# CRIMAC-WP4-Machine-learning/CRIMAC-classifiers-unet

Measured on AMD Instinct MI355X. Metric: echogram patches/sec (4ch 256x256), training step (fwd+weighted CE+bwd+SGD), higher is better.
Workload: dtype bf16; 1 GPU; BASELINE configs[1]: U-Net (depth 5, 64 filters) train step, batch 32 x 4x256x256 per GPU; global_batch=32, precision=bf16, start_filts=64, parallelism=dp1, ranks=1, launcher=single process

## Files before the change

crimac_classifiers_unet_amd/csrc/common.h:

```cpp
#pragma once
#include <hip/hip_runtime.h>
#include <stdint.h>
#include <stdio.h>

#include "../../include/crimac_unet_hip.h"

typedef __bf16 bf16_t;
typedef _Float16 half_t;
typedef _Float16 half8 __attribute__((ext_vector_type(8)));
typedef __bf16 bf16x4 __attribute__((ext_vector_type(4)));
typedef __bf16 bf16x8 __attribute__((ext_vector_type(8)));
typedef unsigned short u16x4 __attribute__((ext_vector_type(4)));
typedef unsigned short u16x8 __attribute__((ext_vector_type(8)));
typedef float f32x4 __attribute__((ext_vector_type(4)));
typedef float f32x16 __attribute__((ext_vector_type(16)));
typedef unsigned int u32x4 __attribute__((ext_vector_type(4)));
typedef unsigned int u32x2 __attribute__((ext_vector_type(2)));

#define LDS_PTR(T) __attribute__((address_space(3))) T*

void crimac_set_error(const char* fmt, ...);
#define CRIMAC_REQUIRE(cond, ...)                 \
  do {                                            \
    if (!(cond)) {                                \
// ... 219 lines not shown
    for (int i = 0; i < 4; ++i) { v[i] = a[i]; v[4 + i] = b[i]; }
  }
#else
  load8(p, v);
#endif
}
__device__ __forceinline__ void store8(bf16_t* p, const float (&v)[8]) {
  u16x8 r;
#pragma unroll
  for (int i = 0; i < 8; ++i) r[i] = f2bfbits(v[i]);
  *reinterpret_cast<u16x8*>(p) = r;
}
__device__ __forceinline__ void store8(half_t* p, const float (&v)[8]) {
  half8 r;
#pragma unroll
  for (int i = 0; i < 8; ++i) r[i] = (half_t)v[i];
  *reinterpret_cast<half8*>(p) = r;
}
__device__ __forceinline__ void store8(float* p, const float (&v)[8]) {
  f32x4 a, b;
#pragma unroll
  for (int i = 0; i < 4; ++i) { a[i] = v[i]; b[i] = v[4 + i]; }
  *reinterpret_cast<f32x4*>(p) = a;
  *reinterpret_cast<f32x4*>(p + 4) = b;
}

__device__ __forceinline__ void store8(hp_t* p, const float (&v)[8]) {
  u32x4 h, l;
  hp_split(v, h, l);
  *reinterpret_cast<u32x4*>(p) = h;
  *(reinterpret_cast<u32x4*>(p) + 1) = l;
}

__device__ __forceinline__ float wave_sum(float v) {
#pragma unroll
  for (int o = 32; o > 0; o >>= 1) v += __shfl_xor(v, o, 64);
  return v;
}
__device__ __forceinline__ double wave_sum_d(double v) {
#pragma unroll
  for (int o = 32; o > 0; o >>= 1) v += __shfl_xor(v, o, 64);
  return v;
}

static inline bool crimac_first_use_on_device(unsigned long long* mask) {
  int dev = 0;
  if (hipGetDevice(&dev) != hipSuccess || dev < 0 || dev >= 64) return true;
  const unsigned long long bit = 1ull << dev;
  return (__atomic_fetch_or(mask, bit, __ATOMIC_ACQ_REL) & bit) == 0;
}
static inline int crimac_cu_count() {
  static int ncu[64] = {0};
  int dev = 0;
  if (hipGetDevice(&dev) != hipSuccess || dev < 0 || dev >= 64) return 256;
  int n = __atomic_load_n(&ncu[dev], __ATOMIC_RELAXED);
  if (n <= 0) {
    hipDeviceProp_t prop;
    n = (hipGetDeviceProperties(&prop, dev) == hipSuccess && prop.multiProcessorCount > 0) ? prop.multiProcessorCount : 256;
    __atomic_store_n(&ncu[dev], n, __ATOMIC_RELAXED);
  }
  return n;
}

#ifdef CRIMAC_DIAG_CLOCK
#define CRIMAC_DIAG_SLOTS 4096
#define CRIMAC_DIAG_DECLARE(name)                                                                   \
// ... 22 lines not shown
```

crimac_classifiers_unet_amd/csrc/elementwise.hip:

```cpp
#include <stdarg.h>
#include <stdlib.h>

#include <mutex>

#include "common.h"

static thread_local char g_err[512] = "";
void crimac_set_error(const char* fmt, ...) {
  va_list ap;
  va_start(ap, fmt);
  vsnprintf(g_err, sizeof(g_err), fmt, ap);
  va_end(ap);
}
extern "C" const char* crimac_last_error(void) { return g_err; }
extern "C" int crimac_version(void) { return CRIMAC_ABI_VERSION; }
extern "C" int crimac_layer_desc_size(void) { return (int)sizeof(crimac_layer_desc); }

namespace {

#ifdef CRIMAC_STREAM_FORWARD
#define CRIMAC_ROW(x, M) (x)
#else
#define CRIMAC_ROW(x, M) ((M) - 1 - (x))
#endif
// ... 813 lines not shown
    load8s(dp + r * dp_ld + c0, g);
    long pix[4];
#pragma unroll
    for (int d = 0; d < 4; ++d) {
      pix[d] = (b * H + 2 * yp + (d >> 1)) * (long)W + 2 * xp + (d & 1);
      load8s(y + pix[d] * y_ld + c0, yv[d]);
#pragma unroll
      for (int j = 0; j < 8; ++j) av[d][j] = storage_round<TA>(fmaxf(yv[d][j] * sc[j] + sh[j], 0.f));
    }
    int arg[8];
#pragma unroll
    for (int j = 0; j < 8; ++j) {
      int best = 0;
      float bv = av[0][j];
#pragma unroll
      for (int d = 1; d < 4; ++d)
        if (av[d][j] > bv) { bv = av[d][j]; best = d; }
      arg[j] = best;
    }
#pragma unroll
    for (int d = 0; d < 4; ++d) {
      float o[8];
      if (ds) load8s(ds + pix[d] * ds_ld + c0, o);
#pragma unroll
      for (int j = 0; j < 8; ++j) {
        const float dav = storage_round<T>((ds ? o[j] : 0.f) + (arg[j] == d ? g[j] : 0.f));
        o[j] = bn_bwd_dy(yv[d][j], dav, sc[j], sh[j], mu[j], is[j], k1[j], k2[j]);
      }
      store8(dy + pix[d] * dy_ld + c0, o);
    }
  }
}

template <typename T, int NC, typename TR = T>
__global__ __launch_bounds__(256) void head_fwd_kernel(const T* __restrict__ x, long x_ld, int Cin,
                                                       const float* __restrict__ w,
                                                       const float* __restrict__ bias,
                                                       float* __restrict__ logits, long npix, long HW,
                                                       int softmax, const float* __restrict__ bn_scale,
                                                       const float* __restrict__ bn_shift) {
  const int lp = Cin / 8;
  const int sub = threadIdx.x % lp;
  float bsc[8], bsh[8];
#pragma unroll
  for (int j = 0; j < 8; ++j) {
    bsc[j] = bn_scale ? bn_scale[sub * 8 + j] : 1.f;
    bsh[j] = bn_scale ? bn_shift[sub * 8 + j] : 0.f;
  }
  float wr[NC][8];
#pragma unroll
  for (int o = 0; o < NC; ++o)
#pragma unroll
    for (int j = 0; j < 8; ++j) wr[o][j] = w[o * Cin + sub * 8 + j];
  const long ppb = 256 / lp;
  for (long p0 = (long)blockIdx.x * ppb; p0 < npix; p0 += (long)gridDim.x * ppb) {
    const long p = p0 + threadIdx.x / lp;
    float acc[NC];
#pragma unroll
    for (int o = 0; o < NC; ++o) acc[o] = 0.f;
    if (p < npix) {
      float v[8];
      load8(x + p * x_ld + sub * 8, v);
      if (bn_scale) {
#pragma unroll
        for (int j = 0; j < 8; ++j) v[j] = storage_round<TR>(fmaxf(v[j] * bsc[j] + bsh[j], 0.f));
      }
// ... 685 lines not shown
  CRIMAC_LAUNCH_CHECK();
  return CRIMAC_OK;
}

extern "C" int crimac_unpool_bn_bwd_apply_replicas(int prec, const void* dp, long dp_ld, const void* ds, long ds_ld,
                                                   const void* y, long y_ld, const float* bn_vec, long bn_stride,
                                                   const double* sum_dz, const double* sum_dz_xhat, int replicas,
                                                   long count, void* dy, long dy_ld, int B, int H, int W, int C,
                                                   float* dgamma, float* dbeta, void* stream) {
  PREC_OK_BWD16("unpool_bn_bwd_apply_replicas");
  CRIMAC_REQUIRE(dp && y && bn_vec && bn_stride >= C && sum_dz && sum_dz_xhat && replicas >= 1 && dy && dgamma && dbeta &&
                     B > 0 && H > 0 && W > 0 && H % 2 == 0 && W % 2 == 0 && C > 0 && C % 8 == 0 && C <= 2048,
                 "unpool_bn_bwd_apply_replicas: bad arguments");
  const long M = (long)B * H * W;
  CRIMAC_REQUIRE(count == 0 || count >= M, "unpool_bn_bwd_apply_replicas: count smaller than the pixels of this call");
  if (count == 0) count = M;
  CRIMAC_REQUIRE(dp_ld >= C && y_ld >= C && dy_ld >= C && (!ds || ds_ld >= C) && dp_ld % 8 == 0 && y_ld % 8 == 0 &&
                     dy_ld % 8 == 0 && (!ds || ds_ld % 8 == 0),
                 "unpool_bn_bwd_apply_replicas: bad pixel strides");
  const long total = (long)B * (H / 2) * (W / 2) * (C / 8);
  const int grid = grid_for(total, 256 * 4);
  const size_t lds = 512 * sizeof(double) + 2 * (size_t)C * sizeof(float);
#define UBA(T, TD, TA)                                                                                                  \
  hipLaunchKernelGGL((unpool_bn_bwd_apply_kernel<T, TD, TA>), dim3(whole_rounds(unpool_bn_bwd_apply_kernel<T, TD, TA>, lds, grid)), dim3(256), lds, ST, (const T*)dp, dp_ld,      \
                     (const T*)ds, ds_ld, (const T*)y, y_ld, bn_vec + 2 * bn_stride, bn_vec + 3 * bn_stride, bn_vec,    \
                     bn_vec + bn_stride, sum_dz, sum_dz_xhat, replicas, count, (TD*)dy, dy_ld, B, H, W, C, dgamma, dbeta)
  if (prec == CRIMAC_PREC_H3F_BWD) UBA(float, half_t, hp_t);
  else CRIMAC_FOR_STORAGE2(prec, T, TP, UBA(T, TP, TP));
#undef UBA
  CRIMAC_LAUNCH_CHECK();
  return CRIMAC_OK;
}

template <typename T, typename TR = T>
static int head_fwd_launch(const void* x, long x_ld, int Cin, const float* w, const float* b,
                           float* logits, long npix, long HW, int ncls, int softmax, const float* bn_scale,
                           const float* bn_shift, hipStream_t st) {
  const int lp = Cin / 8;
  if (Cin == 64) {
    const int grid64 = grid_for(npix, 256 * 4);
#define HF64(NC)                                                                                              \
  hipLaunchKernelGGL((head_fwd64_kernel<T, NC, TR>), dim3(whole_rounds(head_fwd64_kernel<T, NC, TR>, 0, grid64)), dim3(256), 0, st, (const T*)x, x_ld, w, b, logits, \
                     npix, HW, softmax, bn_scale, bn_shift)
    if (ncls == 2) HF64(2); else if (ncls == 3) HF64(3); else HF64(4);
#undef HF64
    CRIMAC_LAUNCH_CHECK();
    return CRIMAC_OK;
  }
  const int grid = grid_for(npix, (256 / lp) * 8);
#define HF(NC)                                                                                      \
  hipLaunchKernelGGL((head_fwd_kernel<T, NC, TR>), dim3(whole_rounds(head_fwd_kernel<T, NC, TR>, 0, grid)), dim3(256), 0, st, (const T*)x, x_ld, Cin, \
                     w, b, logits, npix, HW, softmax, bn_scale, bn_shift)
  if (ncls == 2) HF(2); else if (ncls == 3) HF(3); else HF(4);
#undef HF
  CRIMAC_LAUNCH_CHECK();
  return CRIMAC_OK;
}

static bool head_cin_ok(int Cin) {
  const int lp = Cin / 8;
  return Cin > 0 && Cin % 8 == 0 && lp <= 64 && (lp & (lp - 1)) == 0;
}

extern "C" int crimac_head_fwd(int prec, const void* x, long x_ld, int Cin, const float* w,
                               const float* b, float* logits, int B, int H, int W, int ncls,
                               int softmax, const float* bn_scale, const float* bn_shift, void* stream) {
// ... 137 lines not shown
```

crimac_classifiers_unet_amd/csrc/wgrad.hip:

```cpp
#include "common.h"

CRIMAC_DIAG_DECLARE(crimac_diag_clock_wgrad)

namespace {

struct WgradParams {
  const void* f; long f_ld; int CF;
  const void* s; long s_ld; int CS;
  int B, Hf, Wf;
  float* dw;
  int tiles_y, tiles_x;
  long ntiles;
  int tiles_per_block;
  int nsplits;
  long partial_stride;
  int f_es = 2, s_es = 2;
};

__device__ __forceinline__ int swz_tr(int row) { return ((row >> 1) & 1) << 6; }

__device__ __forceinline__ bf16x4 lds_tr16(const unsigned char* p) {
  return __builtin_amdgcn_ds_read_tr16_b64_v4bf16((LDS_PTR(bf16x4))(p));
}


template <int OFF>
__device__ __forceinline__ bf16x4 lds_tr16_asm(unsigned addr) {
  bf16x4 v;
  asm volatile("ds_read_b64_tr_b16 %0, %1 offset:%2" : "=v"(v) : "v"(addr), "n"(OFF) : "memory");
  return v;
}
template <int N> __device__ __forceinline__ void wait_lgkm() {
  asm volatile("s_waitcnt lgkmcnt(%0)" :: "n"(N) : "memory");
}
__device__ __forceinline__ void tie(bf16x4& x) { asm volatile("" : "+v"(x)); }

__device__ __forceinline__ int swz16(int row) { return (((row >> 1) & 1) << 6) | (((row >> 2) & 1) << 5); }

template <int MODE, int TG>
struct WgTaps {
  static constexpr int TR = MODE == 0 ? 8 : 4;
  static constexpr int NRP = TR / 2;
  static constexpr int RS = MODE == 0 ? 18 : 64;
  static constexpr int T0 = MODE == 0 ? (TG == 0 ? 0 : 5) : (TG == 0 ? 0 : 2);
  static constexpr int N = MODE == 0 ? (TG == 0 ? 5 : 4) : 2;
  static constexpr int srow(int py, int t) {
    return MODE == 0 ? (py + t / 3) * 18 + t % 3 : (2 * py + (t >> 1)) * 32 + (t & 1) * 16;
  }
};
struct WgFrags {
  bf16x4 a[4][2];
  bf16x4 b[2][2][2];
};
template <int RP, int FH>
__device__ __forceinline__ void wg_rd_a(unsigned fv0, WgFrags& f) {
  f.a[FH][0] = lds_tr16_asm<(RP * 32) * 128>(fv0 ^ (FH << 5));
// ... 916 lines not shown
  if (col < 0) {
#else
  if (col < p.CS) {
#endif
    float* dwp = p.dw + (p.partial_stride > 0 ? (long)split * p.partial_stride : 0);
#pragma unroll
    for (int t = 0; t < NTAPS; ++t) {
#pragma unroll
      for (int r = 0; r < 16; ++r) {
        const int row = cf0 + wf * 32 + (r & 3) + 8 * (r >> 2) + 4 * (lane >> 5);
        if (row < p.CF) {
          float* dst = dwp + ((long)t * p.CF + row) * p.CS + col;
          if (p.partial_stride > 0) *dst = acc[t][r];
          else atomicAdd(dst, acc[t][r]);
        }
      }
    }
  }
}

constexpr int kGroupMaxLayers = CRIMAC_WGRAD_GROUP_MAX_LAYERS;
using GroupLayer = crimac_wgrad_group_layer;
struct GroupParams {
  GroupLayer layer[kGroupMaxLayers];
  int B;
  const int* items;
  int cap;
  int count[8];
  unsigned* counter;
  int f_es, s_es;
  int max_items;
};

__device__ __forceinline__ void group_barrier_lds() {
  asm volatile("s_waitcnt lgkmcnt(0)" ::: "memory");
  __builtin_amdgcn_s_barrier();
  asm volatile("" ::: "memory");
}

__device__ __forceinline__ unsigned lds_word(const unsigned* p) {
  return *(volatile LDS_PTR(unsigned))(LDS_PTR(unsigned))(p);
}

template <typename TA>
__global__ __launch_bounds__(512) __attribute__((amdgpu_waves_per_eu(2, 2)))
void wgrad_group_kernel(GroupParams gp) {
  constexpr int MODE = 0, TR = 8, NTAPS = 9;
  constexpr int F_ROWS = TR * 16;
  constexpr int S_ROWS = (TR + 2) * 18;
  constexpr int S_ROWS_PAD = (S_ROWS + 7) / 8 * 8;
  constexpr int F_BYTES = F_ROWS * 128;
  constexpr int S_BYTES = S_ROWS_PAD * 128;
  constexpr int BUF_BYTES = F_BYTES + S_BYTES;
  constexpr int NF = F_ROWS / 8 / 4;
  constexpr int NS = (S_ROWS_PAD / 8 + 3) / 4;
  constexpr unsigned OOB = 0x80000000u;
  extern __shared__ __attribute__((aligned(16))) unsigned char smem[];
  const int tid = threadIdx.x, lane = tid & 63;
  const int team = __builtin_amdgcn_readfirstlane(tid >> 8);
  const int wave = __builtin_amdgcn_readfirstlane((tid >> 6) & 3);
  const int ws = wave & 1, tg = wave >> 1;
  const int g = lane >> 4, li = lane & 15;
  const int q = li >> 2, pp = li & 3;
  const int sub = lane >> 3, c = lane & 7;
  const int xcd = blockIdx.x & 7;
  unsigned* tq = reinterpret_cast<unsigned*>(smem + 4 * BUF_BYTES);
  const int n_items = gp.count[xcd];
  auto fetch_item = [&](int par) {
    const unsigned k = __hip_atomic_fetch_add(gp.counter + xcd, 1u, __ATOMIC_RELAXED, __HIP_MEMORY_SCOPE_AGENT);
    unsigned a = 0, b = 0;
    if (k < (unsigned)n_items) {
// ... 649 lines not shown
```

crimac_classifiers_unet_amd/engine.py:

```python
from __future__ import annotations

import ctypes as C
import os

import torch

from . import hip
from .hip import Act, call, ptr


def _on_device(fn):
    import functools

    @functools.wraps(fn)
    def wrapped(self, *a, **kw):
        if getattr(self, "device", None) is None:
            self.bind()
        dev = self.device
        if dev is None or dev.type != "cuda":
            return fn(self, *a, **kw)
        with torch.cuda.device(dev):
            return fn(self, *a, **kw)
    return wrapped

# ... 409 lines not shown
            return
        arr, bounds = self._layer_table()
        done = getattr(self, "_packed_groups", set())
        if done:
            for gi in range(len(bounds)):
                if gi not in done:
                    self._pack_group(gi)
        elif len(arr):
            call("crimac_pack_layers", C.byref(arr), len(arr), self._fwd_planes_arg())
            if self.bwd16:
                call("crimac_pack_layers", C.byref(self._ltab16), len(arr), hip.PLANES_FP16)
        self._packed_groups = set()
        self._train_pack_dirty = False

    wgrad_side_streams = int(os.environ.get("CRIMAC_WGRAD_STREAM", "1"))
    early_sgd = True
    early_sgd_multi = os.environ.get("CRIMAC_EARLY_SGD_MULTI", "0") != "0"
    exchange_probe = None
    exchange_on_side = os.environ.get("CRIMAC_EXCHANGE_SIDE", "0") != "0"
    _side = None
    _side_events = None
    _eval_side = None

    @staticmethod
    def _gloo_ranks():
        import torch.distributed as dist
        return (dist.is_available() and dist.is_initialized() and dist.get_world_size() > 1
                and dist.get_backend() == "gloo")

    wgrad_group = True
    wgrad_group_h3p = False
    wgrad_group_layers = hip.WGRAD_GROUP_MAX_LAYERS
    _wg_pending = None

    def _groupable(self, prec, mode, cf, cs):
        if not (self.wgrad_group and mode == 0 and cs >= 64 and cf >= 64 and not self.use_wgrad_partials and self._wg_pending is not None):
            return False
        if prec == hip.PREC_H3P:
            return self.wgrad_group_h3p and cf % 64 == 0 and cs % 64 == 0
        return prec in hip.PREC_16BIT or prec == hip.PREC_H3F_BWD

    def _group_plan(self, B, shapes):
        key = (self.prec_bwd, B, shapes)
        plan = self._wg_plans.get(key)
        if plan is None:
            lib = hip.load_library()
            arr = (hip.WgradGroupLayer * len(shapes))()
            for d, (cf, cs, h, w, f_ld, s_ld) in zip(arr, shapes):
                d.CF, d.CS, d.Hf, d.Wf, d.f_ld, d.s_ld = cf, cs, h, w, f_ld, s_ld
            counts = (C.c_int * 8)()
            cap = lib.crimac_wgrad_group_plan(self.prec_bwd, arr, len(shapes), B, 0, None, 0, counts)
            if cap < 0:
                raise hip.HipLibraryError("crimac_wgrad_group_plan failed: " + lib.crimac_last_error().decode(errors="replace"))
            items = torch.zeros(8 * max(cap, 1) * 2, dtype=torch.int32)
            rc = lib.crimac_wgrad_group_plan(self.prec_bwd, arr, len(shapes), B, 0, C.c_void_p(items.data_ptr()), max(cap, 1),
                                             counts)
            if rc < 0:
                raise hip.HipLibraryError("crimac_wgrad_group_plan failed: " + lib.crimac_last_error().decode(errors="replace"))
            plan = (arr, items.to(self.device), counts, max(cap, 1))
            self._wg_plans[key] = plan
        return plan

    def _flush_wgrad_group(self):
        pend = self._wg_pending
        if not pend:
            return
# ... 130 lines not shown
        if t is None or tuple(t.shape) != tuple(shape) or t.dtype != dtype:
            t = torch.empty(shape, dtype=dtype, device=self.device)
            self._bufs[key] = t
        return t

    def _wfrag_geometry(self, B, H, W):
        es = 4 if self.is_hp else 2
        small = (B * H * W - 1) * (2 * self.sf) * es + 2 * self.sf * es < (1 << 31)
        if small == getattr(self, "_wfrag_on", True):
            return
        self._wfrag_on = small
        for pks in (self.pk_main, self.pk_eval, self.pk16):
            for key, pk in pks.items():
                ok = pk.get("frag_ok") or (self.pk_main.get(key, {}).get("frag_ok", (False, False)) if pks is self.pk_eval else None)
                if ok is None:
                    continue
                if "fwd_frag" in pk:
                    pk["fwd_frag"] = bool(small and ok[0])
                if "dg_frag" in pk:
                    pk["dg_frag"] = bool(small and ok[1])
        self._ltab = self._ltab16 = None
        self._packed_groups = set()
        self._train_pack_dirty = self._eval_pack_dirty = True

    def _geom(self, B, H, W):
        self._wfrag_geometry(B, H, W)
        D = self.depth
        if H % (2 ** (D - 1)) or W % (2 ** (D - 1)):
            raise ValueError(f"H, W must be divisible by {2 ** (D - 1)} (got {H}x{W})")
        return [(H >> i, W >> i, B * (H >> i) * (W >> i)) for i in range(D)]

    fuse_bn_bwd = True
    fuse_unpool_apply = None
    fuse_head_bn = True

    def _conv3x3(self, x: Act, pk, bias, out: Act, B, H, W, cin, cout, relu, dgrad=False, cin_real=None,
                 stats=None, bnb=None, cols=None, out_planes=False, stat_reps=None):
        flops = 2.0 * 9 * (cin_real or cin) * cout * B * H * W
        relu = (hip.EPI_RELU if relu else 0) | (hip.EPI_OUT_PLANES if (out_planes and self.is_hp) else 0)
        if pk.get("narrow"):
            return self._conv3x3_narrow(x, pk, bias, out, B, H, W, cin, cout, relu, dgrad, stats, cols, stat_reps, flops)
        if self.is_hp and cin_real is not None and cin_real <= 4 and cin == CIN_PAD and not dgrad:
            relu |= hip.EPI_CIN4
        w_hi, w_lo = ptr(pk["dg_hi" if dgrad else "fwd_hi"]), ptr(pk["dg_lo" if dgrad else "fwd_lo"])
        if pk.get("dg_frag" if dgrad else "fwd_frag"):
            relu |= hip.EPI_WFRAG
        prec = self.prec_bwd if dgrad else self.prec
        mode, s0, s1, by, by_ld, bvec = 0, None, None, None, 0, None
        reps = stat_reps or self._nrep(cout)
        if stats is not None:
            mode, s0, s1 = 1, ptr(stats[0]), ptr(stats[1])
        elif bnb is not None and self.fuse_bn_bwd:
            blk, y = bnb
            mode, s0, s1 = 2, ptr(self._stat(blk, 0)), ptr(self._stat(blk, 1))
            by, by_ld, bvec = y.p, y.ld, ptr(self._bnf(blk, 0))
        if cols is not None:
            call("crimac_conv3x3_cols", prec, x.p, x.ld, B, H, W, cin, cout, w_hi, w_lo, ptr(bias),
                 out.p, out.ld, relu, mode, s0, s1, reps, by, by_ld, bvec, self.cmax,
                 cols[0], cols[1], flops=flops * cols[1] / cout, mfmas=hip.MFMAS_PER_PRODUCT[prec])
            return mode != 0
        call("crimac_conv3x3", prec, x.p, x.ld, B, H, W, cin, cout, w_hi, w_lo, ptr(bias),
             out.p, out.ld, relu, mode, s0, s1, reps, by, by_ld, bvec, self.cmax,
             flops=flops, mfmas=hip.MFMAS_PER_PRODUCT[prec])
        return mode != 0

    def _conv3x3_narrow(self, x: Act, pk, bias, out: Act, B, H, W, cin, cout, flags, dgrad, stats, cols, stat_reps, flops):
# ... 329 lines not shown
            w64, wm = self._lmi_weights()
            call("crimac_head_fwd", self.prec, cur.p, cur.ld, self.sf, ptr(w64), ptr(self.P["conv_final.bias"]),
                 ptr(logits), B, H, W, self.n_classes, 0,
                 ptr(self._bnf(head_bn, 2)) if head_bn is not None else None,
                 ptr(self._bnf(head_bn, 3)) if head_bn is not None else None)
            m = self._buf("lmi.m", (B * H * W,), torch.float32)
            call("crimac_meta_mlp_fwd", ptr(meta), self.meta_channels, B, H, W, *self._mlp(), ptr(m))
            call("crimac_meta_inject_fwd", ptr(m), ptr(wm), ptr(logits), B, H, W, self.n_classes, 1 if softmax else 0)
            saved["meta"] = meta
        else:
            call("crimac_head_fwd", self.prec, cur.p, cur.ld, self.sf, ptr(self.P["conv_final.weight"]),
                 ptr(self.P["conv_final.bias"]), ptr(logits), B, H, W, self.n_classes, 1 if softmax else 0,
                 ptr(self._bnf(head_bn, 2)) if head_bn is not None else None,
                 ptr(self._bnf(head_bn, 3)) if head_bn is not None else None)
        saved["head_in"] = cur if head_bn is None else None
        self.saved = saved if training else None
        if training:
            self.forward_generation += 1
        return logits

    def _block_bwd(self, tag, b, da: Act, y: Act, x_in: Act, B, h, w, M, dx_out: Act, reduce_done=False,
                   next_bn=None, bias_from_stats=None, unpool_src=None):
        world = self._sync_world()
        folded = reduce_done and self.fold_bn_finalize and world == 1
        if folded:
            pass
        elif reduce_done:
            call("crimac_sum_replicas", ptr(self._stat(b, 0)), self._nrep(b.cout), b.cout, b.cout,
                 ptr(self._stat(b, 2)), None, ptr(self._stat(b, 1)), ptr(self._stat(b, 3)))
        else:
            call("crimac_bn_bwd_reduce", self.prec, da.p, da.ld, y.p, y.ld, ptr(self._bnf(b, 2)),
                 ptr(self._bnf(b, 3)), ptr(self._bnf(b, 0)), ptr(self._bnf(b, 1)), M, b.cout,
                 ptr(self._stat(b, 2)), ptr(self._stat(b, 3)))
        dy = Act(self._buf(f"{tag}.dy", (M, b.cout), torch.float16 if self.bwd16 else None), b.cout)
        prec_apply = self.prec_bwd if self.bwd16 else self.prec
        dgamma, dbeta = self.G[b.bn_key + ".weight"], self.G[b.bn_key + ".bias"]
        if world > 1:
            import torch.distributed as dist
            dgamma.copy_(self._stat(b, 3))
            dbeta.copy_(self._stat(b, 2))
            dist.all_reduce(self._stat_pair(b), group=UNetEngine._bn_group)
            scr = self._buf("g.syncbn.scratch", (2, self.cmax), torch.float32)
            dgamma, dbeta = scr[0], scr[1]
        if unpool_src is not None:
            if not folded:
                raise RuntimeError("unpool_src needs the folded BatchNorm-backward path")
            dp_, ds_ = unpool_src
            call("crimac_unpool_bn_bwd_apply_replicas", prec_apply, dp_.p, dp_.ld, ds_.p if ds_ is not None else None,
                 ds_.ld if ds_ is not None else 0, y.p, y.ld, ptr(self._bnf(b, 0)), self.cmax, ptr(self._stat(b, 0)),
                 ptr(self._stat(b, 1)), self._nrep(b.cout), M, dy.p, dy.ld, B, h, w, b.cout, ptr(dgamma), ptr(dbeta))
        elif folded:
            call("crimac_bn_bwd_apply_replicas", prec_apply, da.p, da.ld, y.p, y.ld, ptr(self._bnf(b, 0)), self.cmax,
                 ptr(self._stat(b, 0)), ptr(self._stat(b, 1)), self._nrep(b.cout), M, M, b.cout, dy.p, dy.ld,
                 ptr(dgamma), ptr(dbeta))
        else:
            call("crimac_bn_bwd_apply", prec_apply, da.p, da.ld, y.p, y.ld, ptr(self._bnf(b, 2)),
                 ptr(self._bnf(b, 3)), ptr(self._bnf(b, 0)), ptr(self._bnf(b, 1)), ptr(self._stat(b, 2)),
                 ptr(self._stat(b, 3)), M, M * world, b.cout, dy.p, dy.ld, ptr(dgamma), ptr(dbeta), None)
        self._wgrad(self.prec_bwd, 0, dy.p, dy.ld, b.cout, x_in.p, x_in.ld, b.cin_pad, B, h, w, b.conv_key,
                    flops=2.0 * 9 * b.cin * b.cout * B * h * w)
        fused = False
        if dx_out is not None:
            stats = None
            if bias_from_stats is not None:
                per = 2 * STAT_REPLICAS * 2 * self.cmax
                lvl = bias_from_stats[2]
# ... 81 lines not shown

    def _enc_group(self, i):
        return min(self.depth - i, self.n_enc_groups)

    def grad_ranges(self):
        if getattr(self, "_granges", None) is not None and self._granges[0] is self.layout:
            return self._granges[1]
        r = self._grad_ranges()
        self._granges = (self.layout, r)
        return r

    def _grad_ranges(self):
        dec = self.ups[0].key.split(".")[0] + "."
        lo_dec = min(o for k, (o, _, _) in self.layout.items() if k.startswith(dec))
        starts = {}
        for i in range(self.depth):
            pre = ".".join(self.enc[i][0].conv_key.split(".")[:2]) + "."
            lo = min(o for k, (o, _, _) in self.layout.items() if k.startswith(pre))
            g = self._enc_group(i)
            starts[g] = min(starts.get(g, lo), lo)
        bounds = sorted(starts.items(), key=lambda kv: -kv[1])
        if [g for g, _ in bounds] != sorted(starts) or bounds[-1][1] != 0 or not bounds[0][1] < lo_dec:
            raise RuntimeError("unexpected parameter order in the flat buffer")
        for k, (o, _, _) in self.layout.items():
            if (o >= lo_dec) != (k.startswith(dec) or k.startswith("conv_final") or k.startswith("post_processing_weights")):
                raise RuntimeError(f"unexpected parameter order in the flat buffer at {k}")
        ranges, hi = [(lo_dec, self.n_flat)], lo_dec
        for _, lo in bounds:
            ranges.append((lo, hi))
            hi = lo
        return ranges

    @_on_device
    def backward(self, dlogits, on_ready=None, before_join=None):
        ranges = self.grad_ranges() if on_ready is not None else None
        s = self.saved
        if s is None:
            raise RuntimeError("backward() needs a preceding train-mode forward()")
        B, H, W = s["B"], s["H"], s["W"]
        geo = self._geom(B, H, W)
        D = self.depth
        self._skip_done = {}
        self._unpacked = {}
        self._wg_pending, self._wg_launches = [], 0
        self._dup16 = {}
        self._plan_dw(B, H, W)
        self.flat_g.zero_()
        if not self.use_wgrad_partials:
            self.dw_packed.zero_()
        self.stat[2:].zero_()
        self.bias_scr.zero_()
        dlogits = dlogits.contiguous().float()
        head_in = s["head_in"]
        h, w, M = geo[0]
        d_cur = Act(self._buf("g.head", (M, self.sf)), self.sf)
        head_fused = self.fuse_bn_bwd and D >= 2
        if head_in is None and not head_fused:
            raise RuntimeError("head input was not materialised (fuse_head_bn) but the fused BatchNorm sums are off")
        w_head, g_head = ptr(self.P["conv_final.weight"]), self.G["conv_final.weight"]
        if self.lmi:
            w64, wm = self._lmi_weights()
            g64 = self._buf("lmi.g64", (self.n_classes, self.sf), torch.float32)
            gwm = self._buf("lmi.gwm", (self.n_classes,), torch.float32)
            g64.zero_()
            gwm.zero_()
            pre = "post_processing_weights.main."
            call("crimac_meta_bwd", ptr(dlogits), ptr(s["meta"]), self.meta_channels, B, H, W, self.n_classes, ptr(wm),
                 *self._mlp(), ptr(gwm), *[ptr(self.G[pre + k]) for k in
                                          ("0.weight", "0.bias", "2.weight", "2.bias", "4.weight", "4.bias")])
            w_head, g_head = ptr(w64), g64
        call("crimac_head_bwd", self.prec, ptr(dlogits), head_in.p if head_in is not None else None,
             head_in.ld if head_in is not None else 0, self.sf,
             w_head, d_cur.p, d_cur.ld, ptr(g_head),
             ptr(self.G["conv_final.bias"]), B, H, W, self.n_classes,
             *self._bnb_args(self.dec[D - 2][1], s[f"d{D - 2}"][4] if head_fused else None))
        if self.lmi:
            gw = self.G["conv_final.weight"].view(self.n_classes, self.sf + 1)
            gw[:, :self.sf].copy_(g64)
# ... 138 lines not shown
            self._good_checks += 1
            if self._good_checks >= growth_interval and self.loss_scale < 2.0 ** 24:
                self.loss_scale *= 2.0
                self._good_checks = 0
        return self.loss_scale

    @_on_device
    def train_step(self, x, labels, class_w, lr, momentum, grad_sync=None, ignore_index=-100, meta=None):
        logits = self.forward(x, training=True, meta=meta)
        return self._loss_backward_update(logits, labels, class_w, lr, momentum, grad_sync, ignore_index)

    def _loss_backward_update(self, logits, labels, class_w, lr, momentum, grad_sync, ignore_index):
        sums = self.stat[0:2]
        sums, labels = self.ce_forward(logits, labels, class_w, ignore_index, sums=sums)
        ls = float(self.loss_scale)
        self.last_loss_sums = sums.clone()
        dl = self.ce_backward(logits, labels, class_w, sums, ls, ignore_index)
        scale = 1.0
        single = grad_sync is None or (hasattr(grad_sync, "world") and grad_sync.world() == 1
                                       and not getattr(grad_sync, "force", False))

        def finish_exchange():
            if self.exchange_probe is None:
                return grad_sync.finish()
            e0, e1 = torch.cuda.Event(enable_timing=True), torch.cuda.Event(enable_timing=True)
            e0.record()
            sc = grad_sync.finish()
            e1.record()
            self.exchange_probe.append((e0, e1))
            return sc

        if self.dynamic_loss_scale or ls != 1.0:
            if grad_sync is not None and hasattr(grad_sync, "launch"):
                self.backward(dl, on_ready=None if single else (lambda lo, hi: grad_sync.launch(self.flat_g, lo, hi)))
                scale = finish_exchange()
            else:
                self.backward(dl)
                if grad_sync is not None:
                    scale = grad_sync(self.flat_g)
            self.sgd_step(lr, momentum, grad_scale=scale / ls, guarded=True)
            return (sums[0] / sums[1]).float()
        if single and self.early_sgd and self._side is not None and len(self._side) == 1:
            self._sgd_left = None
            self.mark_dirty()
            self.backward(dl, before_join=lambda: self._early_sgd(lr, momentum))
            for lo, hi in (self._sgd_left if self._sgd_left is not None else [(0, self.n_flat)]):
                self._sgd_range(lo, hi, lr, momentum)
            return (sums[0] / sums[1]).float()
        if grad_sync is not None and hasattr(grad_sync, "launch"):
            self.backward(dl, on_ready=None if single else (lambda lo, hi: grad_sync.launch(self.flat_g, lo, hi)))
            if not single and self.early_sgd and self.early_sgd_multi and hasattr(grad_sync, "finish_range"):
                self.mark_dirty()
                probe = self.exchange_probe is not None
                if probe:
                    e0, e1 = torch.cuda.Event(enable_timing=True), torch.cuda.Event(enable_timing=True)
                    e0.record()
                rngs = self.grad_ranges()
                for g, (lo, hi) in enumerate(rngs):
                    scale = grad_sync.finish_range(lo, hi)
                    if probe and g == len(rngs) - 1:
                        e1.record()
                        self.exchange_probe.append((e0, e1))
                    self._sgd_range(lo, hi, lr, momentum, scale)
                    self._pack_group(g)
                    self._packed_groups.add(g)
                grad_sync.finish()
                return (sums[0] / sums[1]).float()
            scale = finish_exchange()
        else:
            self.backward(dl)
            if grad_sync is not None:
                scale = grad_sync(self.flat_g)
        self.sgd_step(lr, momentum, grad_scale=scale)
        return (sums[0] / sums[1]).float()

    def _early_sgd(self, lr, momentum):
        ranges = self.grad_ranges()
        left = []
        for g, (lo, hi) in enumerate(ranges):
            ev = self._unpacked.get(g)
            if ev is None or g == len(ranges) - 1:
                left.append((lo, hi))
                continue
            torch.cuda.current_stream().wait_event(ev)
            self._sgd_range(lo, hi, lr, momentum)
            self._pack_group(g)
            self._packed_groups.add(g)
        self._sgd_left = left

    def _sgd_range(self, lo, hi, lr, momentum, grad_scale=1.0):
        call("crimac_sgd_momentum", ptr(self.flat_p, lo), ptr(self.flat_g, lo), ptr(self.flat_v, lo), hi - lo,
             float(lr), float(momentum), float(grad_scale), 0)

    @_on_device
    def augment_batch(self, data_linear, labels, seed, do_noise=True, do_flip=True, refine_labels=None, db_scaled=False,
                      n_data=None):
        self.bind()
        if not data_linear.is_cuda:
            raise hip.HipLibraryError("augment_batch: data is not on a GPU")
        data_linear = data_linear.contiguous().float()
        B, C, H, W = data_linear.shape
        if C != self.in_channels:
            raise ValueError(f"expected {self.in_channels} channels, got {C}")
# ... 61 lines not shown
```

include/crimac_unet_hip.h:

```cpp
#ifndef CRIMAC_UNET_HIP_H_
#define CRIMAC_UNET_HIP_H_

#ifdef __cplusplus
extern "C" {
#endif

#define CRIMAC_OK 0
#define CRIMAC_ERR_INVALID (-22)
#define CRIMAC_ERR_LAUNCH (-5)

#define CRIMAC_PREC_BF16 0
#define CRIMAC_PREC_F32X3 1
#define CRIMAC_PREC_F32X6 2
#define CRIMAC_PREC_FP16 3
#define CRIMAC_PREC_F32H3 4
#define CRIMAC_PREC_H3P 5
#define CRIMAC_PREC_MAX 5
#define CRIMAC_PREC_H3F_BWD 6
#define CRIMAC_F32H3_WSHIFT 8
#define CRIMAC_PLANES_FWD_FP16 16
#define CRIMAC_PLANES_DG_FP16 32
#define CRIMAC_PLANES_FP16 (1 | CRIMAC_PLANES_FWD_FP16 | CRIMAC_PLANES_DG_FP16)
#define CRIMAC_PLANES_F32H3 (2 | CRIMAC_PLANES_FWD_FP16 | (CRIMAC_F32H3_WSHIFT << 8))
#define CRIMAC_PLANES_INTERLEAVED 64
#define CRIMAC_PLANES_FWD_FRAG 65536
#define CRIMAC_PLANES_DG_SCALED 128
#define CRIMAC_PLANES_H3P (2 | CRIMAC_PLANES_FWD_FP16 | CRIMAC_PLANES_DG_FP16 | CRIMAC_PLANES_INTERLEAVED | \
                           CRIMAC_PLANES_DG_SCALED | (CRIMAC_F32H3_WSHIFT << 8))

#define CRIMAC_EPI_RELU 1
#define CRIMAC_EPI_OUT_PLANES 2
#define CRIMAC_EPI_CIN4 4
#define CRIMAC_EPI_STAT_RAW 8
#define CRIMAC_EPI_WFRAG 16
#define CRIMAC_EPI_WROWS 32

#define CRIMAC_ABI_VERSION 14
int crimac_version(void);
int crimac_layer_desc_size(void);
const char* crimac_last_error(void);


int crimac_igemm_conv(int prec, const void* in, long in_ld, int B, int Hi, int Wi, int Ho, int Wo,
                      int Cin, int N, int ntaps, int tw, int pad, int stride, const void* w_hi,
                      const void* w_lo, const float* bias, int bias_mod, void* out, long out_ld,
                      int relu, int out_mode, int cout_up, void* stream);

int crimac_upconv2x2_dgrad_bnb(const void* dy, long dy_ld, int B, int H, int W, int Cout, int Cin,
                               const void* w_dg_hi, void* dx, long dx_ld, const void* bnb_y, long bnb_y_ld,
                               const float* bnb_vec, long bnb_stride, double* stat_sum, double* stat_sumsq,
                               int stat_replicas, void* stream);
int crimac_upconv2x2_dgrad_bnb_prec(int prec, const void* dy, long dy_ld, int B, int H, int W, int Cout, int Cin,
                                    const void* w_dg_hi, void* dx, long dx_ld, const void* bnb_y, long bnb_y_ld,
                                    const float* bnb_vec, long bnb_stride, double* stat_sum, double* stat_sumsq,
                                    int stat_replicas, void* stream);


int crimac_conv3x3(int prec, const void* in, long in_ld, int B, int H, int W, int Cin, int N,
                   const void* w_hi, const void* w_lo, const float* bias, void* out, long out_ld,
                   int relu, int stat_mode, double* stat_sum, double* stat_sumsq, int stat_replicas,
                   const void* bnb_y, long bnb_y_ld, const float* bnb_vec, long bnb_stride, void* stream);

int crimac_conv3x3_cols(int prec, const void* in, long in_ld, int B, int H, int W, int Cin, int N,
                   const void* w_hi, const void* w_lo, const float* bias, void* out, long out_ld,
                   int relu, int stat_mode, double* stat_sum, double* stat_sumsq, int stat_replicas,
                   const void* bnb_y, long bnb_y_ld, const float* bnb_vec, long bnb_stride, int n_first, int n_count, void* stream);

int crimac_conv3x3_pool(int prec, const void* in, long in_ld, int B, int H, int W, int Cin, int N,
                        const void* w_hi, const void* w_lo, const float* bias, void* out, long out_ld, int relu,
                        void* pool_out, long pool_ld, void* stream);
// ... 70 lines not shown
                       const float* beta, float eps, float momentum, float* running_mean,
                       float* running_var, long long* num_batches_tracked, float* mean,
                       float* invstd, float* scale, float* shift, void* stream);
int crimac_bn_act_pool(int prec, const void* y, long y_ld, const float* scale, const float* shift,
                       int relu, void* out, long out_ld, void* pool_out, long pool_ld, int B, int H,
                       int W, int C, void* stream);
int crimac_bn_train_act_pool(int prec, const void* y, long y_ld, const double* stat_sum, const double* stat_sumsq,
                             int replicas, long count, const float* gamma, const float* beta, float eps,
                             float momentum, float* running_mean, float* running_var,
                             long long* num_batches_tracked, float* bn_vec, long bn_stride, int relu, void* out,
                             long out_ld, void* pool_out, long pool_ld, int B, int H, int W, int C, void* stream);
int crimac_unpool_add(int prec, const void* dp, long dp_ld, const void* a, long a_ld, const void* ds,
                      long ds_ld, void* da, long da_ld, int B, int H, int W, int C, const void* bnb_y,
                      long bnb_y_ld, const float* bnb_vec, long bnb_stride, double* stat_sum,
                      double* stat_sumsq, int stat_replicas, void* stream);
int crimac_bn_bwd_reduce(int prec, const void* da, long da_ld, const void* y, long y_ld,
                         const float* scale, const float* shift, const float* mean,
                         const float* invstd, long M, int C, double* sum_dz, double* sum_dz_xhat,
                         void* stream);
int crimac_bn_bwd_apply(int prec, const void* da, long da_ld, const void* y, long y_ld,
                        const float* scale, const float* shift, const float* mean, const float* invstd,
                        const double* sum_dz, const double* sum_dz_xhat, long M, long count, int C, void* dy,
                        long dy_ld, float* dgamma, float* dbeta, float* dbias, void* stream);

int crimac_bn_bwd_apply_replicas(int prec, const void* da, long da_ld, const void* y, long y_ld, const float* bn_vec,
                                 long bn_stride, const double* sum_dz, const double* sum_dz_xhat, int replicas, long M,
                                 long count, int C, void* dy, long dy_ld, float* dgamma, float* dbeta, void* stream);

int crimac_unpool_bn_bwd_apply_replicas(int prec, const void* dp, long dp_ld, const void* ds, long ds_ld, const void* y,
                                        long y_ld, const float* bn_vec, long bn_stride, const double* sum_dz,
                                        const double* sum_dz_xhat, int replicas, long count, void* dy, long dy_ld, int B,
                                        int H, int W, int C, float* dgamma, float* dbeta, void* stream);


int crimac_head_fwd(int prec, const void* x, long x_ld, int Cin, const float* w, const float* b,
                    float* logits, int B, int H, int W, int ncls, int softmax, const float* bn_scale,
                    const float* bn_shift, void* stream);
int crimac_head_bwd(int prec, const float* dlogits, const void* x, long x_ld, int Cin, const float* w,
                    void* dx, long dx_ld, float* dw, float* db, int B, int H, int W, int ncls,
                    const void* bnb_y, long bnb_y_ld, const float* bnb_vec, long bnb_stride, double* stat_sum,
                    double* stat_sumsq, int stat_replicas, void* stream);
int crimac_softmax_nchw(const float* logits, float* out, int B, int ncls, int H, int W, void* stream);

int crimac_wce_fwd(const float* logits, const void* labels, int label_bytes, const float* class_w,
                   int ncls, int ignore_index, int B, int H, int W, double* sums, void* stream);
int crimac_wce_bwd(const float* logits, const void* labels, int label_bytes, const float* class_w,
                   int ncls, int ignore_index, int B, int H, int W, const double* sums,
                   float upstream, float* dlogits, void* stream);
int crimac_sgd_momentum(float* p, float* g, float* v, long n, float lr, float momentum,
                        float grad_scale, int zero_grad, void* stream);
int crimac_grad_overflow_flag(const float* g, long n, int* state, void* stream);
int crimac_sgd_momentum_guarded(float* p, float* g, float* v, long n, float lr, float momentum,
                                float grad_scale, int zero_grad, int* state, void* stream);



int crimac_gather_patches(int prec, const float* data, int C, int Wd, int H, const int* centres, int P,
                          int ph, int pw, void* out, long ld, void* stream);
int crimac_gather_patches_memm(int prec, const float* data, int C, int Wd, int H, const int* centres, int P, int ph,
                               int pw, void* out, long ld, const short* border_labels, void* stream);
int crimac_gather_patches_memm_meta(int prec, const float* data, int C, int Wd, int H, const int* centres, int P,
                                    int ph, int pw, void* out, long ld, const short* border_labels, int db_scaled,
                                    int flags, double portion_year, const double* portion_day, int n_day,
                                    const double* time_diff, int n_td, const long long* seabed, int n_sb,
                                    const int* meta_centres, void* stream);
int crimac_gather_patches_memm_labels(int prec, const float* data, int C, int Wd, int H, const int* centres, int P,
// ... 123 lines not shown
```

Measured before the change: 2909 patches/s.

## Fuse first-layer BN backward apply with 3x3 weight-gradient MFMA kernel

Adds a kernel for the first conv layer (4 real input channels padded to 16, 64 outputs) that computes the BN-backward dy tile in registers, stages it in LDS, and feeds it straight into MFMA-based weight-gradient accumulation against a haloed input tile. This removes writing and rereading the full-resolution dy buffer and a separate wgrad launch for the largest-resolution layer. The fused path is used only when dy is not needed (keep_dy=False in train_step) and relies on atomics into dw from every block, with double-buffered register prefetch of the next tile.

```diff
diff --git a/crimac_classifiers_unet_amd/csrc/common.h b/crimac_classifiers_unet_amd/csrc/common.h
--- a/crimac_classifiers_unet_amd/csrc/common.h
+++ b/crimac_classifiers_unet_amd/csrc/common.h
@@ -275,6 +275,15 @@
   *(reinterpret_cast<u32x4*>(p) + 1) = l;
 }
 
+__device__ __forceinline__ bf16x4 lds_tr16(const unsigned char* p) {
+  return __builtin_amdgcn_ds_read_tr16_b64_v4bf16((LDS_PTR(bf16x4))(p));
+}
+__device__ __forceinline__ void barrier_lds() {
+  asm volatile("s_waitcnt lgkmcnt(0)" ::: "memory");
+  __builtin_amdgcn_s_barrier();
+  asm volatile("" ::: "memory");
+}
+
 __device__ __forceinline__ float wave_sum(float v) {
 #pragma unroll
   for (int o = 32; o > 0; o >>= 1) v += __shfl_xor(v, o, 64);
diff --git a/crimac_classifiers_unet_amd/csrc/elementwise.hip b/crimac_classifiers_unet_amd/csrc/elementwise.hip
--- a/crimac_classifiers_unet_amd/csrc/elementwise.hip
+++ b/crimac_classifiers_unet_amd/csrc/elementwise.hip
@@ -869,6 +869,143 @@
   }
 }
 
+constexpr int FLB_X = 256 * 128;
+constexpr int FLB_K12 = FLB_X + 2608;
+constexpr int FLB_LDS = FLB_K12 + 2 * 64 * 4;
+template <typename T>
+__global__ __launch_bounds__(256) void bn_bwd_apply_wgrad_c16_kernel(
+    const T* __restrict__ da, long da_ld, const T* __restrict__ y, long y_ld, const float* __restrict__ scale,
+    const float* __restrict__ shift, const float* __restrict__ mean, const float* __restrict__ invstd,
+    const double* __restrict__ sum_dz, const double* __restrict__ sum_dzx, int nrep, long count, const T* __restrict__ x,
+    long x_ld, int cs_real, int B, int H, int W, float* __restrict__ dw, float* dgamma, float* dbeta) {
+  constexpr int C = 64;
+  constexpr unsigned OOB = 0x80000000u;
+  extern __shared__ __attribute__((aligned(16))) unsigned char fl_smem[];
+  float* k12 = reinterpret_cast<float*>(fl_smem + FLB_K12);
+  const int tid = threadIdx.x, lane = tid & 63;
+  const int wave = __builtin_amdgcn_readfirstlane(tid >> 6);
+  {
+    const double invM = 1.0 / (double)count;
+    const bool writer = blockIdx.x == 0;
+    replica_sums_block(sum_dz, sum_dzx, nrep, C, reinterpret_cast<double*>(fl_smem), [&](int c, double s1, double s2) {
+      k12[c] = (float)(s1 * invM);
+      k12[C + c] = (float)(s2 * invM);
+      if (writer) { dbeta[c] = (float)s1; dgamma[c] = (float)s2; }
+    });
+    __syncthreads();
+  }
+  const int chunk = tid & 7, rl = tid >> 3, c0 = chunk * 8;
+  float sc[8], sh[8], mu[8], is[8], k1[8], k2[8];
+#pragma unroll
+  for (int j = 0; j < 8; ++j) {
+    sc[j] = scale[c0 + j]; sh[j] = shift[c0 + j]; mu[j] = mean[c0 + j]; is[j] = invstd[c0 + j];
+    k1[j] = k12[c0 + j];
+    k2[j] = k12[C + c0 + j];
+  }
+  const int ty0 = rl >> 4, tx = rl & 15;
+  const unsigned da_rel = (unsigned)((((long)ty0 * W + tx) * da_ld + c0) * 2), da_step = (unsigned)(4L * W * da_ld);
+  const unsigned y_rel = (unsigned)((((long)ty0 * W + tx) * y_ld + c0) * 2), y_step = (unsigned)(4L * W * y_ld);
+  const int dy_at = rl * 128 + ((chunk * 16) ^ ((((rl >> 1) & 1) << 6) | (((rl >> 2) & 1) << 5)));
+  int hy[2], hx[2];
+  unsigned x_rel[2];
+#pragma unroll
+  for (int k = 0; k < 2; ++k) {
+    const int e = tid + 256 * k;
+    hy[k] = e / 18;
+    hx[k] = e - hy[k] * 18;
+    x_rel[k] = e < 324 ? (unsigned)((((long)hy[k] * W + hx[k]) * x_ld) * 2) : OOB;
+  }
+  const int g = lane >> 4, li = lane & 15, q = li >> 2, pp = li & 3;
+  const int RF = (g >> 1) * 16 + 4 * (g & 1) + q;
+  const int a_at = RF * 128 + (((wave << 5) + 8 * pp) ^ ((((RF >> 1) & 1) << 6) | (((RF >> 2) & 1) << 5)));
+  int b_at[3];
+#pragma unroll
+  for (int jb = 0; jb < 3; ++jb) {
+    const int t = 4 * jb + pp < 9 ? 4 * jb + pp : 8;
+    b_at[jb] = FLB_X + (((g >> 1) + t / 3) * 18 + 4 * (g & 1) + q + t % 3) * 8;
+  }
+  f32x4 acc[3];
+#pragma unroll
+  for (int jb = 0; jb < 3; ++jb)
+#pragma unroll
+    for (int r = 0; r < 4; ++r) acc[jb][r] = 0.f;
+
+  const int tiles_x = (W + 15) >> 4, tiles_y = (H + 15) >> 4;
+  const int ntiles = B * tiles_y * tiles_x;
+  u32x4 rda[8], ry[8];
+  u32x2 rx[2];
+  int y0 = 0, x0 = 0;
+  auto request = [&](int tile) {
+    const unsigned tt = (unsigned)tile / (unsigned)tiles_x;
+    const long b = tt / (unsigned)tiles_y;
+    y0 = (int)(tt - (unsigned)b * tiles_y) * 16;
+    x0 = (int)((unsigned)tile - tt * tiles_x) * 16;
+    const long pix0 = (b * H + y0) * (long)W + x0;
+    const __amdgpu_buffer_rsrc_t r_da = __builtin_amdgcn_make_buffer_rsrc(const_cast<T*>(da + pix0 * da_ld), 0, 0x7FFFFFFF, 0x00020000);
+    const __amdgpu_buffer_rsrc_t r_y = __builtin_amdgcn_make_buffer_rsrc(const_cast<T*>(y + pix0 * y_ld), 0, 0x7FFFFFFF, 0x00020000);
+    const __amdgpu_buffer_rsrc_t r_x = __builtin_amdgcn_make_buffer_rsrc(const_cast<T*>(x + (pix0 - W - 1) * x_ld), 0, 0x7FFFFFFF, 0x00020000);
+    const bool col_ok = x0 + tx < W;
+#pragma unroll
+    for (int i = 0; i < 8; ++i) {
+      const bool ok = col_ok && y0 + 2 * i + ty0 < H;
+      unsigned o_da = ok ? da_rel + i * da_step : OOB, o_y = ok ? y_rel + i * y_step : OOB;
+      asm("" : "+v"(o_da), "+v"(o_y));
+      rda[i] = __builtin_amdgcn_raw_buffer_load_b128(r_da, (int)o_da, 0, 0);
+      ry[i] = __builtin_amdgcn_raw_buffer_load_b128(r_y, (int)o_y, 0, 0);
+    }
+#pragma unroll
+    for (int k = 0; k < 2; ++k) {
+      const bool ok = (unsigned)(y0 - 1 + hy[k]) < (unsigned)H && (unsigned)(x0 - 1 + hx[k]) < (unsigned)W;
+      unsigned o_x = ok ? x_rel[k] : OOB;
+      asm("" : "+v"(o_x));
+      rx[k] = __builtin_amdgcn_raw_buffer_load_b64(r_x, (int)o_x, 0, 0);
+    }
+  };
+  int tile = ntiles - 1 - (int)blockIdx.x;
+  if (tile >= 0) request(tile);
+  for (; tile >= 0;) {
+    const bool col_ok = x0 + tx < W;
+#pragma unroll
+    for (int i = 0; i < 8; ++i) {
+      const bool ok = col_ok && y0 + 2 * i + ty0 < H;
+      float gv[8], yv[8], o[8];
+      load8(reinterpret_cast<const T*>(&rda[i]), gv);
+      load8(reinterpret_cast<const T*>(&ry[i]), yv);
+#pragma unroll
+      for (int j = 0; j < 8; ++j) {
+        const float v = bn_bwd_dy(yv[j], gv[j], sc[j], sh[j], mu[j], is[j], k1[j], k2[j]);
+        o[j] = ok ? v : 0.f;
+      }
+      store8(reinterpret_cast<T*>(fl_smem + dy_at + 4096 * i), o);
+    }
+    *reinterpret_cast<u32x2*>(fl_smem + FLB_X + 8 * tid) = rx[0];
+    if (tid < 324 - 256) *reinterpret_cast<u32x2*>(fl_smem + FLB_X + 8 * (256 + tid)) = rx[1];
+    tile -= (int)gridDim.x;
+    if (tile >= 0) request(tile);
+    barrier_lds();
+#pragma unroll
+    for (int rp = 0; rp < 8; ++rp) {
+      const bf16x4 a0 = lds_tr16(fl_smem + a_at + rp * 4096), a1 = lds_tr16(fl_smem + a_at + rp * 4096 + 1024);
+      const bf16x8 af = __builtin_shufflevector(a0, a1, 0, 1, 2, 3, 4, 5, 6, 7);
+#pragma unroll
+      for (int jb = 0; jb < 3; ++jb) {
+        const bf16x4 b0 = lds_tr16(fl_smem + b_at[jb] + rp * 288), b1 = lds_tr16(fl_smem + b_at[jb] + rp * 288 + 64);
+        const bf16x8 bfr = __builtin_shufflevector(b0, b1, 0, 1, 2, 3, 4, 5, 6, 7);
+        acc[jb] = E16<T>::mfma16(af, bfr, acc[jb]);
+      }
+    }
+    barrier_lds();
+  }
+#pragma unroll
+  for (int jb = 0; jb < 3; ++jb) {
+    const int t = 4 * jb + (li >> 2), ci = li & 3;
+    if (t < 9 && ci < cs_real) {
+#pragma unroll
+      for (int r = 0; r < 4; ++r) atomicAdd(dw + ((long)t * C + 16 * wave + 4 * g + r) * 16 + ci, acc[jb][r]);
+    }
+  }
+}
+
 template <typename T, int NC, typename TR = T>
 __global__ __launch_bounds__(256) void head_fwd_kernel(const T* __restrict__ x, long x_ld, int Cin,
                                                        const float* __restrict__ w,
@@ -1620,6 +1757,38 @@
   return CRIMAC_OK;
 }
 
+extern "C" int crimac_bn_bwd_apply_wgrad_c16(int prec, const void* da, long da_ld, const void* y, long y_ld,
+                                             const float* bn_vec, long bn_stride, const double* sum_dz,
+                                             const double* sum_dz_xhat, int replicas, long count, int C, const void* x,
+                                             long x_ld, int CS_real, int B, int H, int W, float* dw, float* dgamma,
+                                             float* dbeta, void* stream) {
+  CRIMAC_REQUIRE(prec == CRIMAC_PREC_BF16 || prec == CRIMAC_PREC_FP16, "bn_bwd_apply_wgrad_c16: 16-bit storage only (precision %d)", prec);
+  CRIMAC_REQUIRE(C == 64 && CS_real >= 1 && CS_real <= 4, "bn_bwd_apply_wgrad_c16: 64 output and 1..4 real input channels only (C=%d CS_real=%d)", C, CS_real);
+  CRIMAC_REQUIRE(da && y && bn_vec && bn_stride >= C && sum_dz && sum_dz_xhat && replicas >= 1 && x && dw && dgamma && dbeta &&
+                     B > 0 && H > 0 && W > 0,
+                 "bn_bwd_apply_wgrad_c16: bad arguments");
+  const long M = (long)B * H * W;
+  CRIMAC_REQUIRE(count == 0 || count >= M, "bn_bwd_apply_wgrad_c16: count smaller than the pixels of this call");
+  if (count == 0) count = M;
+  CRIMAC_REQUIRE(da_ld >= C && y_ld >= C && x_ld >= 16 && da_ld % 8 == 0 && y_ld % 8 == 0 && x_ld % 8 == 0,
+                 "bn_bwd_apply_wgrad_c16: bad pixel strides");
+  CRIMAC_REQUIRE(32L * (W + 2) * (da_ld > y_ld ? da_ld : y_ld) < (1L << 31) && 36L * (W + 2) * x_ld < (1L << 31),
+                 "bn_bwd_apply_wgrad_c16: rows too long for the tile addressing");
+  const long ntiles = (long)B * cdiv(H, 16) * cdiv(W, 16);
+  CRIMAC_REQUIRE(ntiles < (1L << 31), "bn_bwd_apply_wgrad_c16: too many tiles");
+  const int grid = (int)(ntiles < kMaxBlocks ? ntiles : kMaxBlocks);
+#define FLB(T)                                                                                                          \
+  hipLaunchKernelGGL((bn_bwd_apply_wgrad_c16_kernel<T>), dim3(whole_rounds(bn_bwd_apply_wgrad_c16_kernel<T>, FLB_LDS, grid)),  \
+                     dim3(256), FLB_LDS, ST, (const T*)da, da_ld, (const T*)y, y_ld, bn_vec + 2 * bn_stride,           \
+                     bn_vec + 3 * bn_stride, bn_vec, bn_vec + bn_stride, sum_dz, sum_dz_xhat, replicas, count,           \
+                     (const T*)x, x_ld, CS_real, B, H, W, dw, dgamma, dbeta)
+  if (prec == CRIMAC_PREC_BF16) FLB(bf16_t);
+  else FLB(half_t);
+#undef FLB
+  CRIMAC_LAUNCH_CHECK();
+  return CRIMAC_OK;
+}
+
 template <typename T, typename TR = T>
 static int head_fwd_launch(const void* x, long x_ld, int Cin, const float* w, const float* b,
                            float* logits, long npix, long HW, int ncls, int softmax, const float* bn_scale,
diff --git a/crimac_classifiers_unet_amd/csrc/wgrad.hip b/crimac_classifiers_unet_amd/csrc/wgrad.hip
--- a/crimac_classifiers_unet_amd/csrc/wgrad.hip
+++ b/crimac_classifiers_unet_amd/csrc/wgrad.hip
@@ -18,10 +18,6 @@
 };
 
 __device__ __forceinline__ int swz_tr(int row) { return ((row >> 1) & 1) << 6; }
-
-__device__ __forceinline__ bf16x4 lds_tr16(const unsigned char* p) {
-  return __builtin_amdgcn_ds_read_tr16_b64_v4bf16((LDS_PTR(bf16x4))(p));
-}
 
 
 template <int OFF>
@@ -1004,11 +1000,7 @@
   int max_items;
 };
 
-__device__ __forceinline__ void group_barrier_lds() {
-  asm volatile("s_waitcnt lgkmcnt(0)" ::: "memory");
-  __builtin_amdgcn_s_barrier();
-  asm volatile("" ::: "memory");
-}
+__device__ __forceinline__ void group_barrier_lds() { barrier_lds(); }
 
 __device__ __forceinline__ unsigned lds_word(const unsigned* p) {
   return *(volatile LDS_PTR(unsigned))(LDS_PTR(unsigned))(p);
diff --git a/crimac_classifiers_unet_amd/engine.py b/crimac_classifiers_unet_amd/engine.py
--- a/crimac_classifiers_unet_amd/engine.py
+++ b/crimac_classifiers_unet_amd/engine.py
@@ -465,6 +465,7 @@
     wgrad_group_h3p = False
     wgrad_group_layers = hip.WGRAD_GROUP_MAX_LAYERS
     _wg_pending = None
+    _keep_dy = True
 
     def _groupable(self, prec, mode, cf, cs):
         if not (self.wgrad_group and mode == 0 and cs >= 64 and cf >= 64 and not self.use_wgrad_partials and self._wg_pending is not None):
@@ -661,6 +662,7 @@
 
     fuse_bn_bwd = True
     fuse_unpool_apply = None
+    fuse_first_layer_bwd = True
     fuse_head_bn = True
 
     def _conv3x3(self, x: Act, pk, bias, out: Act, B, H, W, cin, cout, relu, dgrad=False, cin_real=None,
@@ -1056,6 +1058,13 @@
             call("crimac_bn_bwd_reduce", self.prec, da.p, da.ld, y.p, y.ld, ptr(self._bnf(b, 2)),
                  ptr(self._bnf(b, 3)), ptr(self._bnf(b, 0)), ptr(self._bnf(b, 1)), M, b.cout,
                  ptr(self._stat(b, 2)), ptr(self._stat(b, 3)))
+        if (self.fuse_first_layer_bwd and not self._keep_dy and dx_out is None and folded and unpool_src is None
+                and b.cin_pad == 16 and b.cout == 64 and b.cin <= 4 and self.is16 and not self.bwd16 and not self.use_wgrad_partials):
+            call("crimac_bn_bwd_apply_wgrad_c16", self.prec, da.p, da.ld, y.p, y.ld, ptr(self._bnf(b, 0)), self.cmax,
+                 ptr(self._stat(b, 0)), ptr(self._stat(b, 1)), self._nrep(b.cout), M, b.cout, x_in.p, x_in.ld, b.cin,
+                 B, h, w, ptr(self._dw(b.conv_key)[0]), ptr(self.G[b.bn_key + ".weight"]), ptr(self.G[b.bn_key + ".bias"]),
+                 flops=2.0 * 9 * b.cin * b.cout * B * h * w, mfmas=hip.MFMAS_PER_PRODUCT[self.prec_bwd])
+            return False
         dy = Act(self._buf(f"{tag}.dy", (M, b.cout), torch.float16 if self.bwd16 else None), b.cout)
         prec_apply = self.prec_bwd if self.bwd16 else self.prec
         dgamma, dbeta = self.G[b.bn_key + ".weight"], self.G[b.bn_key + ".bias"]
@@ -1203,7 +1212,7 @@
         return ranges
 
     @_on_device
-    def backward(self, dlogits, on_ready=None, before_join=None):
+    def backward(self, dlogits, on_ready=None, before_join=None, keep_dy=True):
         ranges = self.grad_ranges() if on_ready is not None else None
         s = self.saved
         if s is None:
@@ -1215,6 +1224,7 @@
         self._unpacked = {}
         self._wg_pending, self._wg_launches = [], 0
         self._dup16 = {}
+        self._keep_dy = keep_dy
         self._plan_dw(B, H, W)
         self.flat_g.zero_()
         if not self.use_wgrad_partials:
@@ -1419,10 +1429,10 @@
 
         if self.dynamic_loss_scale or ls != 1.0:
             if grad_sync is not None and hasattr(grad_sync, "launch"):
-                self.backward(dl, on_ready=None if single else (lambda lo, hi: grad_sync.launch(self.flat_g, lo, hi)))
+                self.backward(dl, keep_dy=False, on_ready=None if single else (lambda lo, hi: grad_sync.launch(self.flat_g, lo, hi)))
                 scale = finish_exchange()
             else:
-                self.backward(dl)
+                self.backward(dl, keep_dy=False)
                 if grad_sync is not None:
                     scale = grad_sync(self.flat_g)
             self.sgd_step(lr, momentum, grad_scale=scale / ls, guarded=True)
@@ -1430,12 +1440,12 @@
         if single and self.early_sgd and self._side is not None and len(self._side) == 1:
             self._sgd_left = None
             self.mark_dirty()
-            self.backward(dl, before_join=lambda: self._early_sgd(lr, momentum))
+            self.backward(dl, keep_dy=False, before_join=lambda: self._early_sgd(lr, momentum))
             for lo, hi in (self._sgd_left if self._sgd_left is not None else [(0, self.n_flat)]):
                 self._sgd_range(lo, hi, lr, momentum)
             return (sums[0] / sums[1]).float()
         if grad_sync is not None and hasattr(grad_sync, "launch"):
-            self.backward(dl, on_ready=None if single else (lambda lo, hi: grad_sync.launch(self.flat_g, lo, hi)))
+            self.backward(dl, keep_dy=False, on_ready=None if single else (lambda lo, hi: grad_sync.launch(self.flat_g, lo, hi)))
             if not single and self.early_sgd and self.early_sgd_multi and hasattr(grad_sync, "finish_range"):
                 self.mark_dirty()
                 probe = self.exchange_probe is not None
@@ -1455,7 +1465,7 @@
                 return (sums[0] / sums[1]).float()
             scale = finish_exchange()
         else:
-            self.backward(dl)
+            self.backward(dl, keep_dy=False)
             if grad_sync is not None:
                 scale = grad_sync(self.flat_g)
         self.sgd_step(lr, momentum, grad_scale=scale)
diff --git a/include/crimac_unet_hip.h b/include/crimac_unet_hip.h
--- a/include/crimac_unet_hip.h
+++ b/include/crimac_unet_hip.h
@@ -35,7 +35,7 @@
 #define CRIMAC_EPI_WFRAG 16
 #define CRIMAC_EPI_WROWS 32
 
-#define CRIMAC_ABI_VERSION 14
+#define CRIMAC_ABI_VERSION 15
 int crimac_version(void);
 int crimac_layer_desc_size(void);
 const char* crimac_last_error(void);
@@ -172,6 +172,11 @@
                                         const double* sum_dz_xhat, int replicas, long count, void* dy, long dy_ld, int B,
                                         int H, int W, int C, float* dgamma, float* dbeta, void* stream);
 
+int crimac_bn_bwd_apply_wgrad_c16(int prec, const void* da, long da_ld, const void* y, long y_ld, const float* bn_vec,
+                                  long bn_stride, const double* sum_dz, const double* sum_dz_xhat, int replicas, long count,
+                                  int C, const void* x, long x_ld, int CS_real, int B, int H, int W, float* dw,
+                                  float* dgamma, float* dbeta, void* stream);
+
 
 int crimac_head_fwd(int prec, const void* x, long x_ld, int Cin, const float* w, const float* b,
                     float* logits, int B, int H, int W, int ncls, int softmax, const float* bn_scale,
```

Measured after the change: 2915 patches/s, median of 4. Within noise of the previous version (+0.2%).
